# google/kubeflow

Measured on AMD Instinct MI355X. Metric: pytorchjob_train_tokens_per_s, higher is better.
Workload: dtype bf16; 1 GPU; model=llama3-8b, global_batch=7, seq_len=4096, parallelism=dp1

## Files before the change

kubeflow_amd/ops/__init__.py:

```python
from __future__ import annotations

import ctypes
import os
from typing import Optional

import torch

from . import reference
from . import _backend

__all__ = [
    "rms_norm", "layer_norm", "rope", "flash_attention", "attention_decode",
    "flash_attention_rect", "skinny_linear", "kv_store",
    "decode_rope_store", "skinny_linear_q8", "quantize_fp8_rows",
    "dequantize_fp8_rows",
    "cross_entropy", "fused_adamw", "rope_cos_sin", "native_available",
    "masked_attention",
    "swiglu", "fused_qkv_attention",
]

rope_cos_sin = reference.rope_cos_sin


def native_available() -> bool:
# ... 446 lines not shown
    def backward(ctx, dy):
        lib = _backend.require()
        (h2,) = ctx.saved_tensors
        T, F2 = h2.shape
        dy2 = dy.contiguous().view(T, F2 // 2)
        dh = torch.empty_like(h2)
        _backend.check(lib.kf_swiglu_bwd(_p(dh), _p(dy2), _p(h2), T, F2 // 2,
                                         _stream()), "swiglu_bwd")
        return dh.view(ctx.shape)


def swiglu(h: torch.Tensor) -> torch.Tensor:
    if _use_native(h):
        return _SwigluHip.apply(h)
    g, u = h.chunk(2, dim=-1)
    return torch.nn.functional.silu(g) * u



class _FusedQkvAttentionHip(torch.autograd.Function):

    @staticmethod
    def forward(ctx, qkv, cos, sin, Hq, Hkv, D, causal, scale):
        lib = _backend.require()
        B, S, _ = qkv.shape
        ts = (Hq + 2 * Hkv) * D
        qkv = qkv.contiguous()
        _backend.check(
            lib.kf_rope(_p(qkv), _p_off(qkv, Hq * D), _fp(cos), _fp(sin),
                        _ip_or_null(None), B, S, Hq, Hkv, D, ts, ts, 0, 0,
                        _stream()), "rope_fwd")
        o = torch.empty(B, S, Hq * D, dtype=qkv.dtype, device=qkv.device)
        lse = torch.empty(B, Hq, S, dtype=torch.float32, device=qkv.device)
        _backend.check(
            lib.kf_attn_fwd(_p(o), _fp(lse), _p(qkv), _p_off(qkv, Hq * D),
                            _p_off(qkv, (Hq + Hkv) * D), B, S, Hq, Hkv, D,
                            ts, ts, float(scale), int(causal), _stream()),
            "attn_fwd")
        ctx.save_for_backward(qkv, cos, sin, o, lse)
        ctx.meta = (Hq, Hkv, D, causal, scale)
        return o

    @staticmethod
    def backward(ctx, dout):
        lib = _backend.require()
        qkv, cos, sin, o, lse = ctx.saved_tensors
        Hq, Hkv, D, causal, scale = ctx.meta
        B, S, _ = qkv.shape
        ts = (Hq + 2 * Hkv) * D
        dout = dout.contiguous()
        dqkv = torch.empty_like(qkv)
        delta = torch.empty(B, Hq, S, dtype=torch.float32, device=qkv.device)
        _backend.check(
            lib.kf_attn_bwd(_p(dqkv), _p_off(dqkv, Hq * D),
                            _p_off(dqkv, (Hq + Hkv) * D), _p(dout), _p(qkv),
                            _p_off(qkv, Hq * D), _p_off(qkv, (Hq + Hkv) * D),
                            _p(o), _fp(lse), _fp(delta), B, S, Hq, Hkv, D,
                            ts, ts, ts, ts, float(scale), int(causal),
                            _stream()), "attn_bwd")
        _backend.check(
            lib.kf_rope(_p(dqkv), _p_off(dqkv, Hq * D), _fp(cos), _fp(sin),
                        _ip_or_null(None), B, S, Hq, Hkv, D, ts, ts, 0, 1,
                        _stream()), "rope_bwd")
        return dqkv, None, None, None, None, None, None, None


def fused_qkv_attention(qkv: torch.Tensor, cos: torch.Tensor,
                        sin: torch.Tensor, Hq: int, Hkv: int, D: int,
                        causal: bool = True,
                        scale: Optional[float] = None) -> torch.Tensor:
    if scale is None:
        scale = D ** -0.5
    B, S, _ = qkv.shape
    if _use_native(qkv) and S % 128 == 0:
        return _FusedQkvAttentionHip.apply(qkv, cos, sin, Hq, Hkv, D, causal,
                                           scale)
    q, k, v = qkv.split([Hq * D, Hkv * D, Hkv * D], dim=-1)
    q = q.reshape(B, S, Hq, D)
    k = k.reshape(B, S, Hkv, D)
    v = v.reshape(B, S, Hkv, D)
    q, k = rope(q, k, cos, sin)
    o = flash_attention(q, k, v, causal=causal, scale=scale)
    return o.reshape(B, S, Hq * D)



class _LayerNormHip(torch.autograd.Function):
    @staticmethod
    def forward(ctx, x, weight, bias, eps):
        lib = _backend.require()
        shape = x.shape
        x2 = x.contiguous().view(-1, shape[-1])
        rows, cols = x2.shape
        y = torch.empty_like(x2)
        mu = torch.empty(rows, dtype=torch.float32, device=x.device)
        rstd = torch.empty(rows, dtype=torch.float32, device=x.device)
        _backend.check(
            lib.kf_layernorm_fwd(_p(y), _fp(mu), _fp(rstd), _p(x2), _p(weight),
                                 _p(bias), rows, cols, float(eps), _stream()),
            "layernorm_fwd")
        ctx.save_for_backward(x2, weight, mu, rstd)
        ctx.shape = shape
        return y.view(shape)

    @staticmethod
    def backward(ctx, dy):
        lib = _backend.require()
        x2, weight, mu, rstd = ctx.saved_tensors
        rows, cols = x2.shape
        dy2 = dy.contiguous().view(rows, cols)
        dx = torch.empty_like(x2)
        dw = torch.empty_like(weight)
        db = torch.empty_like(weight)
        part = torch.zeros(2 * cols, dtype=torch.float32, device=x2.device)
        _backend.check(
            lib.kf_layernorm_bwd(_p(dx), _p(dw), _p(db), _fp(part), _p(dy2),
# ... 120 lines not shown
```

kubeflow_amd/ops/_backend.py:

```python
from __future__ import annotations

import ctypes
import os
from pathlib import Path

_LIB_PATH = Path(__file__).resolve().parent / "libkfops.so"
_lib = None
_load_error: str | None = None


def native_enabled() -> bool:
    return os.environ.get("KF_NATIVE_KERNELS", "1") != "0"


def try_load():
    global _lib, _load_error
    if _lib is not None:
        return _lib
    if not native_enabled():
        _load_error = "disabled via KF_NATIVE_KERNELS=0"
        return None
    from . import build_ext
    if build_ext.needs_build():
        try:
# ... 13 lines not shown
def require():
    lib = try_load()
    if lib is None:
        raise RuntimeError(
            "kubeflow_amd native kernels unavailable on a GPU machine: "
            f"{_load_error}. Build with `python -m kubeflow_amd.ops.build_ext` "
            "or set KF_NATIVE_KERNELS=0 to explicitly allow the (slow) "
            "reference path.")
    return lib


def _configure(lib: ctypes.CDLL) -> None:
    c = ctypes
    P, F, I64, I32, FP = c.c_void_p, c.c_float, c.c_int64, c.c_int, c.POINTER(c.c_float)
    PI64 = c.POINTER(c.c_int64)
    PI32 = c.POINTER(c.c_int32)
    lib.kf_rmsnorm_fwd.restype = I32
    lib.kf_rmsnorm_fwd.argtypes = [P, FP, P, P, I64, I64, F, P]
    lib.kf_rmsnorm_bwd.restype = I32
    lib.kf_rmsnorm_bwd.argtypes = [P, P, FP, P, P, P, FP, I64, I64, P]
    lib.kf_rmsnorm_bwd_nparts.restype = I64
    lib.kf_rmsnorm_bwd_nparts.argtypes = [I64]
    lib.kf_rope.restype = I32
    lib.kf_rope.argtypes = [P, P, FP, FP, PI64, I64, I64, I64, I64, I64, I64, I64, I64, I32, P]
    lib.kf_adamw.restype = I32
    lib.kf_adamw.argtypes = [P, FP, P, FP, FP, FP, I64, F, F, F, F, F, I64, P]
    lib.kf_ce_fwd.restype = I32
    lib.kf_ce_fwd.argtypes = [FP, FP, P, PI64, I64, I64, I64, P]
    lib.kf_ce_bwd.restype = I32
    lib.kf_ce_bwd.argtypes = [P, P, FP, PI64, FP, I64, I64, I64, P]
    lib.kf_attn_fwd.restype = I32
    lib.kf_attn_fwd.argtypes = [P, FP, P, P, P, I64, I64, I64, I64, I64, I64, I64, F, I32, P]
    if hasattr(lib, "kf_skinny_gemm"):
        lib.kf_skinny_gemm.restype = I32
        lib.kf_skinny_gemm.argtypes = [P, P, P, P, FP, F, I64, I64, I64,
                                       I64, I64, I64, I64, P]
    if hasattr(lib, "kf_skinny_gemm_q8"):
        lib.kf_skinny_gemm_q8.restype = I32
        lib.kf_skinny_gemm_q8.argtypes = [P, P, P, FP, P, FP, F, I64,
                                          I64, I64, I64, I64, I64, I64,
                                          P]
    if hasattr(lib, "kf_kv_store"):
        lib.kf_kv_store.restype = I32
        lib.kf_kv_store.argtypes = [P, P, P, P, P, P, I64, I64, I64, P]
    if hasattr(lib, "kf_attn_fwd4_rect"):
        lib.kf_attn_fwd4_rect.restype = I32
        lib.kf_attn_fwd4_rect.argtypes = [P, FP, P, P, P, I64, I64, I64,
                                          I64, I64, I64, I64, I64, F, I64, P]
    if hasattr(lib, "kf_attn_bwd"):
        lib.kf_attn_bwd.restype = I32
        lib.kf_attn_bwd.argtypes = [P, P, P, P, P, P, P, P, FP, FP, I64, I64,
                                    I64, I64, I64, I64, I64, I64, I64, F, I32,
                                    P]
    lib.kf_layernorm_fwd.restype = I32
    lib.kf_layernorm_fwd.argtypes = [P, FP, FP, P, P, P, I64, I64, F, P]
    lib.kf_layernorm_bwd.restype = I32
    lib.kf_layernorm_bwd.argtypes = [P, P, P, FP, P, P, P, FP, FP, I64, I64, P]
    lib.kf_layernorm_bwd_nparts.restype = I64
    lib.kf_layernorm_bwd_nparts.argtypes = [I64]
    lib.kf_swiglu_fwd.restype = I32
    lib.kf_swiglu_fwd.argtypes = [P, P, I64, I64, P]
    lib.kf_swiglu_bwd.restype = I32
    lib.kf_swiglu_bwd.argtypes = [P, P, P, I64, I64, P]
    lib.kf_attn_decode.restype = I32
    lib.kf_attn_decode.argtypes = [P, P, P, P, P, P, PI32, PI32, I64, I64,
                                   I64, I64, I64, I64, F, P]
    if hasattr(lib, "kf_decode_rope_store"):
        lib.kf_decode_rope_store.restype = I32
        lib.kf_decode_rope_store.argtypes = [P, P, P, P, FP, FP, PI32, P,
                                             I64, I64, I64, I64, I64, P]


def check(err: int, name: str) -> None:
    if err != 0:
        raise RuntimeError(f"HIP kernel {name} failed with hipError_t={err}")
```

kubeflow_amd/ops/csrc/attention_bwd.hip:

```cpp

#include "kf_common.h"

typedef __bf16 kf_bf16x8 __attribute__((ext_vector_type(8)));
typedef float kf_f32x4 __attribute__((ext_vector_type(4)));

#define AB_D 128

__device__ __forceinline__ int kf_swz2(int row, int byte_in_row, int row_bytes,
                                       int xor_mask) {
  return row * row_bytes + (byte_in_row ^ ((row & xor_mask) << 4));
}

__global__ __launch_bounds__(256) void kf_attn_delta2_kernel(
    float* __restrict__ delta, const unsigned short* __restrict__ dout,
    const unsigned short* __restrict__ o, int64_t B, int S, int Hq) {
  const int64_t nrows = B * (int64_t)S * Hq;
  const int wid = threadIdx.x / KF_WAVE;
  const int lane = threadIdx.x & (KF_WAVE - 1);
  for (int64_t row = blockIdx.x * 4 + wid; row < nrows; row += gridDim.x * 4) {
    const unsigned short* dor = dout + row * AB_D;
    const unsigned short* orow = o + row * AB_D;
    kf_short4 a = *reinterpret_cast<const kf_short4*>(dor + lane * 2);
    kf_short4 bv = *reinterpret_cast<const kf_short4*>(orow + lane * 2);
    float s = kf_bf16_to_f32((unsigned short)a[0]) *
// ... 251 lines not shown
                        : __expf(st[nt][r] * scale - lse_c);
          float ds = p * (dpt[nt][r] - dlt_c) * scale;
          const int prow = lg * 4 + r;
          *reinterpret_cast<unsigned short*>(
              pt_lds[w] + kf_swz2(prow, (nt * 16 + l16) * 2, 64, 3)) =
              kf_f32_to_bf16(p);
          *reinterpret_cast<unsigned short*>(
              dst_lds[w] + kf_swz2(prow, (nt * 16 + l16) * 2, 64, 3)) =
              kf_f32_to_bf16(ds);
        }
      }
      __builtin_amdgcn_s_waitcnt(0);

      kf_bf16x8 ptf = *reinterpret_cast<const kf_bf16x8*>(
          pt_lds[w] + kf_swz2(l16, lg * 16, 64, 3));
      kf_bf16x8 dstf = *reinterpret_cast<const kf_bf16x8*>(
          dst_lds[w] + kf_swz2(l16, lg * 16, 64, 3));
#pragma unroll
      for (int nt = 0; nt < 8; ++nt) {
        kf_bf16x8 dob = *reinterpret_cast<const kf_bf16x8*>(
            dot_lds + kf_swz2(nt * 16 + l16, lg * 16, 64, 3));
        dvacc[nt] =
            __builtin_amdgcn_mfma_f32_16x16x32_bf16(ptf, dob, dvacc[nt], 0, 0, 0);
        kf_bf16x8 qb = *reinterpret_cast<const kf_bf16x8*>(
            qt_lds + kf_swz2(nt * 16 + l16, lg * 16, 64, 3));
        dkacc[nt] =
            __builtin_amdgcn_mfma_f32_16x16x32_bf16(dstf, qb, dkacc[nt], 0, 0, 0);
      }
    }
  }

  const int krow0 = kt * 64 + w * 16 + lg * 4;
#pragma unroll
  for (int r = 0; r < 4; ++r) {
    const int64_t base = (b * S + krow0 + r) * dkts + (int64_t)hkv * AB_D;
#pragma unroll
    for (int nt = 0; nt < 8; ++nt) {
      dk[base + nt * 16 + l16] = kf_f32_to_bf16(dkacc[nt][r]);
      dv[base + nt * 16 + l16] = kf_f32_to_bf16(dvacc[nt][r]);
    }
  }
}

extern "C" int kf_attn_bwd8_dq(void*, const void*, const void*, const void*,
                               const void*, const float*, const float*,
                               int64_t, int64_t, int64_t, int64_t, int64_t,
                               int64_t, int64_t, float, int, void*);
extern "C" int kf_attn_bwd8_dkv(void*, void*, const void*, const void*,
                                const void*, const void*, const float*,
                                const float*, int64_t, int64_t, int64_t,
                                int64_t, int64_t, int64_t, int64_t, float,
                                int, void*);

KF_EXPORT int kf_attn_bwd(void* dq, void* dk, void* dv, const void* dout,
                          const void* q, const void* k, const void* v,
                          const void* o, const float* lse, float* delta,
                          int64_t B, int64_t S, int64_t Hq, int64_t Hkv,
                          int64_t D, int64_t qts, int64_t kts, int64_t dqts,
                          int64_t dkts, float scale, int causal,
                          void* stream) {
  if (D != AB_D || S % 64 || Hq % Hkv) return (int)hipErrorInvalidValue;
  if (qts == 0) qts = Hq * AB_D;
  if (kts == 0) kts = Hkv * AB_D;
  if (dqts == 0) dqts = Hq * AB_D;
  if (dkts == 0) dkts = Hkv * AB_D;
  hipLaunchKernelGGL(kf_attn_delta2_kernel,
                     dim3(kf_grid_for(B * S * Hq, 4)), dim3(256), 0,
                     (hipStream_t)stream, delta, (const unsigned short*)dout,
                     (const unsigned short*)o, B, (int)S, (int)Hq);
  int err = (int)hipGetLastError();
  if (err) return err;
  if (S % 256 == 0) {
    err = kf_attn_bwd8_dq(dq, q, k, v, dout, lse, delta, B, S, Hq, Hkv, qts,
                          kts, dqts, scale, causal, stream);
    if (err) return err;
    return kf_attn_bwd8_dkv(dk, dv, q, k, v, dout, lse, delta, B, S, Hq, Hkv,
                            qts, kts, dkts, scale, causal, stream);
  }
  dim3 gq((unsigned)(S / 64), (unsigned)Hq, (unsigned)B);
  hipLaunchKernelGGL(kf_attn_dq_kernel, gq, dim3(256), 0, (hipStream_t)stream,
                     (unsigned short*)dq, (const unsigned short*)q,
                     (const unsigned short*)k, (const unsigned short*)v,
                     (const unsigned short*)dout, lse, delta, B, (int)S,
                     (int)Hq, (int)Hkv, qts, kts, dqts, scale, causal);
  err = (int)hipGetLastError();
  if (err) return err;
  dim3 gkv((unsigned)(S / 64), (unsigned)Hkv, (unsigned)B);
  hipLaunchKernelGGL(kf_attn_dkv_kernel, gkv, dim3(256), 0,
                     (hipStream_t)stream, (unsigned short*)dk,
                     (unsigned short*)dv, (const unsigned short*)q,
                     (const unsigned short*)k, (const unsigned short*)v,
                     (const unsigned short*)dout, lse, delta, B, (int)S,
                     (int)Hq, (int)Hkv, qts, kts, dkts, scale, causal);
  return (int)hipGetLastError();
}
```

kubeflow_amd/ops/csrc/attention_bwd8.hip:

```cpp

#include "kf_common.h"

typedef __bf16 kf_bf16x8 __attribute__((ext_vector_type(8)));
typedef float kf_f32x16 __attribute__((ext_vector_type(16)));
typedef short kf_short4b __attribute__((ext_vector_type(4)));

#define AB_D 128
#define AB_LOG2E 1.44269504f

__device__ __forceinline__ int kf_vsub8(int r, int d) {
  return ((d >> 4) << 10) + ((r >> 2) << 6) + ((r & 3) << 4) + (d & 15);
}

__device__ __forceinline__ int kf_subrow8(int r, int byte_in_row) {
  return 2 * kf_vsub8(r, byte_in_row >> 1);
}

__device__ __forceinline__ unsigned int kf_cvt_pk_bf16b(float lo, float hi) {
  unsigned int r;
  asm volatile("v_cvt_pk_bf16_f32 %0, %1, %2" : "=v"(r) : "v"(lo), "v"(hi));
  return r;
}

__device__ __forceinline__ float kf_exp2b(float x) {
  float r;
  asm volatile("v_exp_f32 %0, %1" : "=v"(r) : "v"(x));
  return r;
}

#define KF_TR16_B(dst, addr, OFFLIT)                                    \
  asm volatile("ds_read_b64_tr_b16 %0, %1 offset:" OFFLIT               \
               : "=v"(dst) : "v"(addr))

__device__ __forceinline__ kf_bf16x8 kf_exchange8(const kf_f32x16& a,
                                                  int base) {
  unsigned int w0 = kf_cvt_pk_bf16b(a[base + 0], a[base + 1]);
  unsigned int w1 = kf_cvt_pk_bf16b(a[base + 2], a[base + 3]);
  unsigned int w2 = kf_cvt_pk_bf16b(a[base + 4], a[base + 5]);
  unsigned int w3 = kf_cvt_pk_bf16b(a[base + 6], a[base + 7]);
  auto s02 = __builtin_amdgcn_permlane32_swap(w0, w2, false, false);
  auto s13 = __builtin_amdgcn_permlane32_swap(w1, w3, false, false);
  unsigned int u[4] = {(unsigned)s02[0], (unsigned)s13[0], (unsigned)s02[1],
                       (unsigned)s13[1]};
  return *reinterpret_cast<kf_bf16x8*>(u);
}

__device__ __forceinline__ unsigned kf_tr_lane_off(int lane) {
  const int g = lane >> 4;
  return (unsigned)(((g & 1) << 11) + ((g >> 1) << 8) + ((lane & 15) << 3));
}

#define KF_TR_ACC_LOOP(acc, vbase, pb0, pb1)                                 \
  {                                                                          \
    kf_short4b t_[2][4];                                                     \
    KF_TR16_B(t_[0][0], (vbase), "0");                                       \
    KF_TR16_B(t_[0][1], (vbase), "128");                                     \
    KF_TR16_B(t_[0][2], (vbase), "512");                                     \
    KF_TR16_B(t_[0][3], (vbase), "640");                                     \
    _Pragma("unroll") for (int dt = 0; dt < 4; ++dt) {                       \
      if (dt < 3) {                                                          \
        const unsigned va_ = (vbase) + ((dt + 1) << 12);                     \
        KF_TR16_B(t_[(dt + 1) & 1][0], va_, "0");                            \
        KF_TR16_B(t_[(dt + 1) & 1][1], va_, "128");                          \
        KF_TR16_B(t_[(dt + 1) & 1][2], va_, "512");                          \
        KF_TR16_B(t_[(dt + 1) & 1][3], va_, "640");                          \
        asm volatile("s_waitcnt lgkmcnt(4)" ::: "memory");                   \
      } else {                                                               \
        asm volatile("s_waitcnt lgkmcnt(0)" ::: "memory");                   \
      }                                                                      \
      __builtin_amdgcn_sched_barrier(0);                                     \
      kf_short8 f0_ = __builtin_shufflevector(t_[dt & 1][0], t_[dt & 1][1],  \
                                              0, 1, 2, 3, 4, 5, 6, 7);       \
      kf_short8 f1_ = __builtin_shufflevector(t_[dt & 1][2], t_[dt & 1][3],  \
                                              0, 1, 2, 3, 4, 5, 6, 7);       \
      __builtin_amdgcn_s_setprio(1);                                         \
      acc[dt] = __builtin_amdgcn_mfma_f32_32x32x16_bf16(                     \
          *reinterpret_cast<kf_bf16x8*>(&f0_), (pb0), acc[dt], 0, 0, 0);     \
      acc[dt] = __builtin_amdgcn_mfma_f32_32x32x16_bf16(                     \
          *reinterpret_cast<kf_bf16x8*>(&f1_), (pb1), acc[dt], 0, 0, 0);     \
      __builtin_amdgcn_s_setprio(0);                                         \
    }                                                                        \
  }

#define KF_TR_ACC_LOOP_B(acc, vbase, pa0, pa1)                               \
  {                                                                          \
    kf_short4b t_[2][4];                                                     \
    KF_TR16_B(t_[0][0], (vbase), "0");                                       \
    KF_TR16_B(t_[0][1], (vbase), "128");                                     \
    KF_TR16_B(t_[0][2], (vbase), "512");                                     \
    KF_TR16_B(t_[0][3], (vbase), "640");                                     \
    _Pragma("unroll") for (int dt = 0; dt < 4; ++dt) {                       \
      if (dt < 3) {                                                          \
        const unsigned va_ = (vbase) + ((dt + 1) << 12);                     \
        KF_TR16_B(t_[(dt + 1) & 1][0], va_, "0");                            \
        KF_TR16_B(t_[(dt + 1) & 1][1], va_, "128");                          \
        KF_TR16_B(t_[(dt + 1) & 1][2], va_, "512");                          \
        KF_TR16_B(t_[(dt + 1) & 1][3], va_, "640");                          \
        asm volatile("s_waitcnt lgkmcnt(4)" ::: "memory");                   \
      } else {                                                               \
        asm volatile("s_waitcnt lgkmcnt(0)" ::: "memory");                   \
      }                                                                      \
      __builtin_amdgcn_sched_barrier(0);                                     \
      kf_short8 f0_ = __builtin_shufflevector(t_[dt & 1][0], t_[dt & 1][1],  \
                                              0, 1, 2, 3, 4, 5, 6, 7);       \
      kf_short8 f1_ = __builtin_shufflevector(t_[dt & 1][2], t_[dt & 1][3],  \
                                              0, 1, 2, 3, 4, 5, 6, 7);       \
      __builtin_amdgcn_s_setprio(1);                                         \
      acc[dt] = __builtin_amdgcn_mfma_f32_32x32x16_bf16(                     \
          (pa0), *reinterpret_cast<kf_bf16x8*>(&f0_), acc[dt], 0, 0, 0);     \
      acc[dt] = __builtin_amdgcn_mfma_f32_32x32x16_bf16(                     \
          (pa1), *reinterpret_cast<kf_bf16x8*>(&f1_), acc[dt], 0, 0, 0);     \
      __builtin_amdgcn_s_setprio(0);                                         \
    }                                                                        \
  }

#define DQ8_QT 256
#define DQ8_KT 64

__global__ __launch_bounds__(512, 2) void kf_attn_dq8_kernel(
    unsigned short* __restrict__ dq, const unsigned short* __restrict__ q,
    const unsigned short* __restrict__ k, const unsigned short* __restrict__ v,
    const unsigned short* __restrict__ dout, const float* __restrict__ lse,
    const float* __restrict__ delta, int64_t B, int S, int Hq, int Hkv,
    int64_t qts, int64_t kts, int64_t dqts, float scale, int causal) {
  __shared__ unsigned char k_lds[2][DQ8_KT * AB_D * 2];
  __shared__ unsigned char v_lds[2][DQ8_KT * AB_D * 2];

  const int nqt = gridDim.x / (Hq * (int)B);
  const int qt = causal ? (nqt - 1 - blockIdx.x / (Hq * (int)B))
                        : (int)(blockIdx.x / (Hq * (int)B));
  const int rest = blockIdx.x % (Hq * (int)B);
  const int hq = rest % Hq;
  const int64_t b = rest / Hq;
  const int hkv = hq / (Hq / Hkv);
  const int tid = threadIdx.x;
  const int w = tid / KF_WAVE;
  const int lane = tid & 63, l31 = lane & 31, hi = lane >> 5;
  const int qrow_g = qt * DQ8_QT + w * 32 + l31;
  const int wave_qmax = qt * DQ8_QT + w * 32 + 31;
  const float scale2 = scale * AB_LOG2E;

  kf_bf16x8 qfrag[8], dofrag[8];
  {
    const int64_t qb = (b * S + qrow_g) * qts + (int64_t)hq * AB_D;
    const int64_t db = ((b * S + qrow_g) * (int64_t)Hq + hq) * AB_D;
#pragma unroll
    for (int kk = 0; kk < 8; ++kk) {
      qfrag[kk] =
          *reinterpret_cast<const kf_bf16x8*>(q + qb + kk * 16 + hi * 8);
      dofrag[kk] =
          *reinterpret_cast<const kf_bf16x8*>(dout + db + kk * 16 + hi * 8);
    }
  }
  const float lse2_q =
      lse[(b * Hq + hq) * (int64_t)S + qrow_g] * AB_LOG2E;
  const float dlt_q = delta[(b * Hq + hq) * (int64_t)S + qrow_g];

  kf_f32x16 dqacc[4];
#pragma unroll
  for (int i = 0; i < 4; ++i) dqacc[i] = kf_f32x16{0.f};

  const unsigned short* kg0 = k + (b * S) * kts + (int64_t)hkv * AB_D;
  const unsigned short* vg0 = v + (b * S) * kts + (int64_t)hkv * AB_D;
  const int sr0 = tid >> 4, sr1 = (tid + 512) >> 4, c8 = tid & 15;
  const unsigned tr_off = kf_tr_lane_off(lane);

  const int last_kt =
      causal ? (qt * DQ8_QT + DQ8_QT - 1) / DQ8_KT : (S / DQ8_KT - 1);

  kf_short8 kst0, kst1, vst0, vst1;
  kst0 = *reinterpret_cast<const kf_short8*>(kg0 + sr0 * kts + c8 * 8);
  kst1 = *reinterpret_cast<const kf_short8*>(kg0 + sr1 * kts + c8 * 8);
  vst0 = *reinterpret_cast<const kf_short8*>(vg0 + sr0 * kts + c8 * 8);
  vst1 = *reinterpret_cast<const kf_short8*>(vg0 + sr1 * kts + c8 * 8);
  *reinterpret_cast<kf_short8*>(k_lds[0] + 2 * kf_vsub8(sr0, c8 * 8)) = kst0;
  *reinterpret_cast<kf_short8*>(k_lds[0] + 2 * kf_vsub8(sr1, c8 * 8)) = kst1;
  *reinterpret_cast<kf_short8*>(v_lds[0] + 2 * kf_vsub8(sr0, c8 * 8)) = vst0;
// ... 17 lines not shown
      const int kv_lo = kt * DQ8_KT + mt * 32;
      if (causal && kv_lo > wave_qmax) continue;
      kf_f32x16 st = kf_f32x16{0.f}, dpt = kf_f32x16{0.f};
      __builtin_amdgcn_s_setprio(1);
#pragma unroll
      for (int kk = 0; kk < 8; ++kk) {
        kf_bf16x8 ka = *reinterpret_cast<const kf_bf16x8*>(
            k_lds[cur] + kf_subrow8(mt * 32 + l31, kk * 32 + hi * 16));
        st = __builtin_amdgcn_mfma_f32_32x32x16_bf16(ka, qfrag[kk], st, 0, 0,
                                                     0);
        kf_bf16x8 va = *reinterpret_cast<const kf_bf16x8*>(
            v_lds[cur] + kf_subrow8(mt * 32 + l31, kk * 32 + hi * 16));
        dpt = __builtin_amdgcn_mfma_f32_32x32x16_bf16(va, dofrag[kk], dpt, 0,
                                                      0, 0);
      }
      __builtin_amdgcn_s_setprio(0);

      const int kv0 = kv_lo + hi * 4;
      const bool need_mask = causal && kv_lo + 31 > qt * DQ8_QT + w * 32;
      if (need_mask) {
#pragma unroll
        for (int r = 0; r < 16; ++r) {
          const int kv = kv0 + (r & 3) + 8 * (r >> 2);
          const float p = (kv > qrow_g)
                              ? 0.f
                              : kf_exp2b(st[r] * scale2 - lse2_q);
          st[r] = p * (dpt[r] - dlt_q) * scale;
        }
      } else {
#pragma unroll
        for (int r = 0; r < 16; ++r) {
          const float p = kf_exp2b(st[r] * scale2 - lse2_q);
          st[r] = p * (dpt[r] - dlt_q) * scale;
        }
      }
      kf_bf16x8 pb0 = kf_exchange8(st, 0), pb1 = kf_exchange8(st, 8);
      const unsigned vbase =
          (unsigned)(size_t)(k_lds[cur]) + tr_off + (mt << 10);
      KF_TR_ACC_LOOP(dqacc, vbase, pb0, pb1);
    }

    if (have_next) {
      const int nxt = cur ^ 1;
      *reinterpret_cast<kf_short8*>(k_lds[nxt] + 2 * kf_vsub8(sr0, c8 * 8)) =
          kst0;
      *reinterpret_cast<kf_short8*>(k_lds[nxt] + 2 * kf_vsub8(sr1, c8 * 8)) =
          kst1;
      *reinterpret_cast<kf_short8*>(v_lds[nxt] + 2 * kf_vsub8(sr0, c8 * 8)) =
          vst0;
      *reinterpret_cast<kf_short8*>(v_lds[nxt] + 2 * kf_vsub8(sr1, c8 * 8)) =
          vst1;
    }
    __syncthreads();
  }

  const int64_t dqb = (b * S + qrow_g) * dqts + (int64_t)hq * AB_D;
#pragma unroll
  for (int dt = 0; dt < 4; ++dt)
#pragma unroll
    for (int rq = 0; rq < 4; ++rq) {
      const int d0 = dt * 32 + 8 * rq + 4 * hi;
      unsigned short q4[4];
#pragma unroll
      for (int j = 0; j < 4; ++j)
        q4[j] = kf_f32_to_bf16(dqacc[dt][rq * 4 + j]);
      *reinterpret_cast<kf_short4b*>(dq + dqb + d0) =
          *reinterpret_cast<kf_short4b*>(q4);
    }
}

#define DKV8_KT 256
#define DKV8_QT 64

__global__ __launch_bounds__(512, 2) void kf_attn_dv8_kernel(
    unsigned short* __restrict__ dv, const unsigned short* __restrict__ q,
    const unsigned short* __restrict__ k,
    const unsigned short* __restrict__ dout, const float* __restrict__ lse,
    int64_t B, int S, int Hq, int Hkv, int64_t qts, int64_t kts,
    int64_t dkts, float scale, int causal) {
  __shared__ unsigned char q_lds[2][DKV8_QT * AB_D * 2];
  __shared__ unsigned char dot_lds[2][DKV8_QT * AB_D * 2];
  __shared__ float lse_s[2][DKV8_QT];

  const int kt = blockIdx.x / (Hkv * (int)B);
  const int rest = blockIdx.x % (Hkv * (int)B);
  const int hkv = rest % Hkv;
  const int64_t b = rest / Hkv;
  const int g = Hq / Hkv;
  const int tid = threadIdx.x;
  const int w = tid / KF_WAVE;
  const int lane = tid & 63, l31 = lane & 31, hi = lane >> 5;
  const int kvrow_g = kt * DKV8_KT + w * 32 + l31;
  const int wave_kv_min = kt * DKV8_KT + w * 32;
  const float scale2 = scale * AB_LOG2E;

  const unsigned short* kvb_k =
      k + (b * S + kvrow_g) * kts + (int64_t)hkv * AB_D;
  kf_bf16x8 kbf[8];
#pragma unroll
  for (int kk = 0; kk < 8; ++kk)
    kbf[kk] =
        *reinterpret_cast<const kf_bf16x8*>(kvb_k + kk * 16 + hi * 8);

  kf_f32x16 dvacc[4];
#pragma unroll
  for (int i = 0; i < 4; ++i) dvacc[i] = kf_f32x16{0.f};
// ... 52 lines not shown
      __builtin_amdgcn_s_setprio(1);
#pragma unroll
      for (int kk = 0; kk < 8; ++kk) {
        kf_bf16x8 qa = *reinterpret_cast<const kf_bf16x8*>(
            q_lds[cur] + kf_subrow8(mt * 32 + l31, kk * 32 + hi * 16));
        sacc = __builtin_amdgcn_mfma_f32_32x32x16_bf16(qa, kbf[kk], sacc, 0,
                                                       0, 0);
      }
      __builtin_amdgcn_s_setprio(0);

      const int q0 = mt * 32 + hi * 4;
      const bool need_mask = causal && q_lo <= kt * DKV8_KT + w * 32 + 31;
      if (need_mask) {
#pragma unroll
        for (int r = 0; r < 16; ++r) {
          const int ql = q0 + (r & 3) + 8 * (r >> 2);
          const int qq = qt * DKV8_QT + ql;
          sacc[r] = (kvrow_g > qq)
                        ? 0.f
                        : kf_exp2b(sacc[r] * scale2 - lse_s[cur][ql]);
        }
      } else {
#pragma unroll
        for (int r = 0; r < 16; ++r) {
          const int ql = q0 + (r & 3) + 8 * (r >> 2);
          sacc[r] = kf_exp2b(sacc[r] * scale2 - lse_s[cur][ql]);
        }
      }
      kf_bf16x8 pa0 = kf_exchange8(sacc, 0), pa1 = kf_exchange8(sacc, 8);
      const unsigned vbase =
          (unsigned)(size_t)(dot_lds[cur]) + tr_off + (mt << 10);
      KF_TR_ACC_LOOP_B(dvacc, vbase, pa0, pa1);
    }
    if (have_next) stage_write(cur ^ 1);
    __syncthreads();
  }

  const int kvbase = kt * DKV8_KT + w * 32 + hi * 4;
#pragma unroll
  for (int r = 0; r < 16; ++r) {
    const int kvr = kvbase + (r & 3) + 8 * (r >> 2);
    const int64_t base = (b * S + kvr) * dkts + (int64_t)hkv * AB_D;
#pragma unroll
    for (int dt = 0; dt < 4; ++dt)
      dv[base + dt * 32 + l31] = kf_f32_to_bf16(dvacc[dt][r]);
  }
}

__global__ __launch_bounds__(512, 2) void kf_attn_dk8_kernel(
    unsigned short* __restrict__ dk, const unsigned short* __restrict__ q,
    const unsigned short* __restrict__ k, const unsigned short* __restrict__ v,
    const unsigned short* __restrict__ dout, const float* __restrict__ lse,
    const float* __restrict__ delta, int64_t B, int S, int Hq, int Hkv,
    int64_t qts, int64_t kts, int64_t dkts, float scale, int causal) {
  __shared__ unsigned char q_lds[2][DKV8_QT * AB_D * 2];
  __shared__ unsigned char do_lds[2][DKV8_QT * AB_D * 2];
  __shared__ float lse_s2[2][DKV8_QT], dlt_s2[2][DKV8_QT];

  const int kt = blockIdx.x / (Hkv * (int)B);
  const int rest = blockIdx.x % (Hkv * (int)B);
  const int hkv = rest % Hkv;
  const int64_t b = rest / Hkv;
  const int g = Hq / Hkv;
  const int tid = threadIdx.x;
  const int w = tid / KF_WAVE;
  const int lane = tid & 63, l31 = lane & 31, hi = lane >> 5;
  const int kvrow_g = kt * DKV8_KT + w * 32 + l31;
  const int wave_kv_min = kt * DKV8_KT + w * 32;
  const float scale2 = scale * AB_LOG2E;

  const unsigned short* kvb_k =
      k + (b * S + kvrow_g) * kts + (int64_t)hkv * AB_D;
  const unsigned short* kvb_v =
      v + (b * S + kvrow_g) * kts + (int64_t)hkv * AB_D;
  kf_bf16x8 kbf[8], vbf[8];
#pragma unroll
  for (int kk = 0; kk < 8; ++kk) {
    kbf[kk] =
        *reinterpret_cast<const kf_bf16x8*>(kvb_k + kk * 16 + hi * 8);
    vbf[kk] =
        *reinterpret_cast<const kf_bf16x8*>(kvb_v + kk * 16 + hi * 8);
  }

  kf_f32x16 dkacc[4];
#pragma unroll
  for (int i = 0; i < 4; ++i) dkacc[i] = kf_f32x16{0.f};

  const int qt0 = causal ? (kt * DKV8_KT) / DKV8_QT : 0;
  const int nqt = S / DKV8_QT;
  const int per_head = nqt - qt0;
  const int total = g * per_head;
  const int sr0 = tid >> 4, sr1 = (tid + 512) >> 4, c8 = tid & 15;
  const unsigned tr_off = kf_tr_lane_off(lane);

  kf_short8 sq0, sq1, sd0, sd1;
  float lse_ld = 0.f, dlt_ld = 0.f;
  auto stage_load = [&](int flat) {
    const int hq = hkv * g + flat / per_head;
    const int qt = qt0 + flat % per_head;
    const unsigned short* qg =
        q + (b * S + qt * DKV8_QT) * qts + (int64_t)hq * AB_D;
    const unsigned short* dog =
        dout + ((b * S + qt * DKV8_QT) * (int64_t)Hq + hq) * AB_D;
    if (tid < DKV8_QT)
      lse_ld = lse[(b * Hq + hq) * (int64_t)S + qt * DKV8_QT + tid];
    else if (tid < 2 * DKV8_QT)
      dlt_ld =
// ... 31 lines not shown
    for (int mt = 0; mt < 2; ++mt) {
      const int q_lo = qt * DKV8_QT + mt * 32;
      if (causal && q_lo + 31 < wave_kv_min) continue;
      kf_f32x16 sacc = kf_f32x16{0.f}, dpacc = kf_f32x16{0.f};
      __builtin_amdgcn_s_setprio(1);
#pragma unroll
      for (int kk = 0; kk < 8; ++kk) {
        kf_bf16x8 qa = *reinterpret_cast<const kf_bf16x8*>(
            q_lds[cur] + kf_subrow8(mt * 32 + l31, kk * 32 + hi * 16));
        sacc = __builtin_amdgcn_mfma_f32_32x32x16_bf16(qa, kbf[kk], sacc, 0,
                                                       0, 0);
        kf_bf16x8 da = *reinterpret_cast<const kf_bf16x8*>(
            do_lds[cur] + kf_subrow8(mt * 32 + l31, kk * 32 + hi * 16));
        dpacc = __builtin_amdgcn_mfma_f32_32x32x16_bf16(da, vbf[kk], dpacc,
                                                        0, 0, 0);
      }
      __builtin_amdgcn_s_setprio(0);

      const int q0 = mt * 32 + hi * 4;
      const bool need_mask = causal && q_lo <= kt * DKV8_KT + w * 32 + 31;
      if (need_mask) {
#pragma unroll
        for (int r = 0; r < 16; ++r) {
          const int ql = q0 + (r & 3) + 8 * (r >> 2);
          const int qq = qt * DKV8_QT + ql;
          const float p =
              (kvrow_g > qq)
                  ? 0.f
                  : kf_exp2b(sacc[r] * scale2 - lse_s2[cur][ql]);
          sacc[r] = p * (dpacc[r] - dlt_s2[cur][ql]) * scale;
        }
      } else {
#pragma unroll
        for (int r = 0; r < 16; ++r) {
          const int ql = q0 + (r & 3) + 8 * (r >> 2);
          const float p = kf_exp2b(sacc[r] * scale2 - lse_s2[cur][ql]);
          sacc[r] = p * (dpacc[r] - dlt_s2[cur][ql]) * scale;
        }
      }
      kf_bf16x8 ds0 = kf_exchange8(sacc, 0), ds1 = kf_exchange8(sacc, 8);
      const unsigned vbase =
          (unsigned)(size_t)(q_lds[cur]) + tr_off + (mt << 10);
      KF_TR_ACC_LOOP_B(dkacc, vbase, ds0, ds1);
    }
    if (have_next) stage_write(cur ^ 1);
    __syncthreads();
  }

  const int kvbase = kt * DKV8_KT + w * 32 + hi * 4;
#pragma unroll
  for (int r = 0; r < 16; ++r) {
    const int kvr = kvbase + (r & 3) + 8 * (r >> 2);
    const int64_t base = (b * S + kvr) * dkts + (int64_t)hkv * AB_D;
#pragma unroll
    for (int dt = 0; dt < 4; ++dt)
      dk[base + dt * 32 + l31] = kf_f32_to_bf16(dkacc[dt][r]);
  }
}

KF_EXPORT int kf_attn_bwd8_dq(void* dq, const void* q, const void* k,
                              const void* v, const void* dout,
                              const float* lse, const float* delta, int64_t B,
                              int64_t S, int64_t Hq, int64_t Hkv, int64_t qts,
                              int64_t kts, int64_t dqts, float scale,
                              int causal, void* stream) {
  dim3 gq((unsigned)((S / DQ8_QT) * Hq * B), 1, 1);
  hipLaunchKernelGGL(kf_attn_dq8_kernel, gq, dim3(512), 0,
                     (hipStream_t)stream, (unsigned short*)dq,
                     (const unsigned short*)q, (const unsigned short*)k,
                     (const unsigned short*)v, (const unsigned short*)dout,
                     lse, delta, B, (int)S, (int)Hq, (int)Hkv, qts, kts, dqts,
                     scale, causal);
  return (int)hipGetLastError();
}

KF_EXPORT int kf_attn_bwd8_dkv(void* dk, void* dv, const void* q,
                               const void* k, const void* v, const void* dout,
                               const float* lse, const float* delta,
                               int64_t B, int64_t S, int64_t Hq, int64_t Hkv,
                               int64_t qts, int64_t kts, int64_t dkts,
                               float scale, int causal, void* stream) {
  dim3 gkv((unsigned)((S / DKV8_KT) * Hkv * B), 1, 1);
  hipLaunchKernelGGL(kf_attn_dv8_kernel, gkv, dim3(512), 0,
                     (hipStream_t)stream, (unsigned short*)dv,
                     (const unsigned short*)q, (const unsigned short*)k,
                     (const unsigned short*)dout, lse, B, (int)S, (int)Hq,
                     (int)Hkv, qts, kts, dkts, scale, causal);
  int err = (int)hipGetLastError();
  if (err) return err;
  hipLaunchKernelGGL(kf_attn_dk8_kernel, gkv, dim3(512), 0,
                     (hipStream_t)stream, (unsigned short*)dk,
                     (const unsigned short*)q, (const unsigned short*)k,
                     (const unsigned short*)v, (const unsigned short*)dout,
                     lse, delta, B, (int)S, (int)Hq, (int)Hkv, qts, kts,
                     dkts, scale, causal);
  return (int)hipGetLastError();
}
```

Baseline: 21070 tokens/s.

## Fuse RoPE backward into attention backward and merge dK/dV kernels

Applies the inverse RoPE rotation to dQ and dK inside the attention backward epilogues, which removes the separate rope backward kernel and its extra read/write pass over dqkv. It also adds a fused dK+dV kernel, now the default, that computes S and dP once per tile and accumulates both gradients. Previously two separate kernels each recomputed the QK^T products and reloaded Q/dO. The fused kernel keeps V in LDS and uses more registers (launch bounds of 2), so occupancy may drop. An environment variable switches back to the old split path.

```diff
diff --git a/kubeflow_amd/ops/__init__.py b/kubeflow_amd/ops/__init__.py
--- a/kubeflow_amd/ops/__init__.py
+++ b/kubeflow_amd/ops/__init__.py
@@ -522,16 +522,14 @@
         dqkv = torch.empty_like(qkv)
         delta = torch.empty(B, Hq, S, dtype=torch.float32, device=qkv.device)
         _backend.check(
-            lib.kf_attn_bwd(_p(dqkv), _p_off(dqkv, Hq * D),
-                            _p_off(dqkv, (Hq + Hkv) * D), _p(dout), _p(qkv),
-                            _p_off(qkv, Hq * D), _p_off(qkv, (Hq + Hkv) * D),
-                            _p(o), _fp(lse), _fp(delta), B, S, Hq, Hkv, D,
-                            ts, ts, ts, ts, float(scale), int(causal),
-                            _stream()), "attn_bwd")
-        _backend.check(
-            lib.kf_rope(_p(dqkv), _p_off(dqkv, Hq * D), _fp(cos), _fp(sin),
-                        _ip_or_null(None), B, S, Hq, Hkv, D, ts, ts, 0, 1,
-                        _stream()), "rope_bwd")
+            lib.kf_attn_bwd_rope(_p(dqkv), _p_off(dqkv, Hq * D),
+                                 _p_off(dqkv, (Hq + Hkv) * D), _p(dout),
+                                 _p(qkv), _p_off(qkv, Hq * D),
+                                 _p_off(qkv, (Hq + Hkv) * D), _p(o),
+                                 _fp(lse), _fp(delta), B, S, Hq, Hkv, D,
+                                 ts, ts, ts, ts, float(scale), int(causal),
+                                 _fp(cos), _fp(sin), 0, _stream()),
+            "attn_bwd_rope")
         return dqkv, None, None, None, None, None, None, None
 
 
diff --git a/kubeflow_amd/ops/_backend.py b/kubeflow_amd/ops/_backend.py
--- a/kubeflow_amd/ops/_backend.py
+++ b/kubeflow_amd/ops/_backend.py
@@ -89,6 +89,21 @@
         lib.kf_attn_bwd.argtypes = [P, P, P, P, P, P, P, P, FP, FP, I64, I64,
                                     I64, I64, I64, I64, I64, I64, I64, F, I32,
                                     P]
+    if hasattr(lib, "kf_attn_bwd_rope"):
+        lib.kf_attn_bwd_rope.restype = I32
+        lib.kf_attn_bwd_rope.argtypes = [P, P, P, P, P, P, P, P, FP, FP, I64,
+                                         I64, I64, I64, I64, I64, I64, I64,
+                                         I64, F, I32, FP, FP, I64, P]
+    dq8 = [P, P, P, P, P, FP, FP, I64, I64, I64, I64, I64, I64, I64, F, I32]
+    dkv8 = [P] + dq8
+    for name, args in (("kf_attn_bwd8_dq", dq8), ("kf_attn_bwd8_dkv", dkv8),
+                       ("kf_attn_bwd8_dkv_fused", dkv8)):
+        if hasattr(lib, name):
+            getattr(lib, name).restype = I32
+            getattr(lib, name).argtypes = args + [P]
+        if hasattr(lib, name + "_rope"):
+            getattr(lib, name + "_rope").restype = I32
+            getattr(lib, name + "_rope").argtypes = args + [FP, FP, I64, P]
     lib.kf_layernorm_fwd.restype = I32
     lib.kf_layernorm_fwd.argtypes = [P, FP, FP, P, P, P, I64, I64, F, P]
     lib.kf_layernorm_bwd.restype = I32
diff --git a/kubeflow_amd/ops/csrc/attention_bwd.hip b/kubeflow_amd/ops/csrc/attention_bwd.hip
--- a/kubeflow_amd/ops/csrc/attention_bwd.hip
+++ b/kubeflow_amd/ops/csrc/attention_bwd.hip
@@ -327,6 +327,49 @@
                                 int64_t, int64_t, int64_t, int64_t, float,
                                 int, void*);
 
+extern "C" int kf_attn_bwd8_dq_rope(void*, const void*, const void*,
+                                    const void*, const void*, const float*,
+                                    const float*, int64_t, int64_t, int64_t,
+                                    int64_t, int64_t, int64_t, int64_t, float,
+                                    int, const float*, const float*, int64_t,
+                                    void*);
+extern "C" int kf_attn_bwd8_dkv_rope(void*, void*, const void*, const void*,
+                                     const void*, const void*, const float*,
+                                     const float*, int64_t, int64_t, int64_t,
+                                     int64_t, int64_t, int64_t, int64_t,
+                                     float, int, const float*, const float*,
+                                     int64_t, void*);
+extern "C" int kf_attn_bwd8_dkv_fused_rope(void*, void*, const void*,
+                                           const void*, const void*,
+                                           const void*, const float*,
+                                           const float*, int64_t, int64_t,
+                                           int64_t, int64_t, int64_t, int64_t,
+                                           int64_t, float, int, const float*,
+                                           const float*, int64_t, void*);
+
+extern "C" int kf_rope(void*, void*, const float*, const float*,
+                       const int64_t*, int64_t, int64_t, int64_t, int64_t,
+                       int64_t, int64_t, int64_t, int64_t, int, void*);
+
+static int kf_attn_bwd_impl() {
+  static int cached = -1;
+  if (cached < 0) {
+    const char* e = getenv("KF_ATTN_BWD_IMPL");
+    cached = (e && e[0] == '1') ? 1 : 2;
+  }
+  return cached;
+}
+
+KF_EXPORT int kf_attn_bwd_rope(void* dq, void* dk, void* dv, const void* dout,
+                               const void* q, const void* k, const void* v,
+                               const void* o, const float* lse, float* delta,
+                               int64_t B, int64_t S, int64_t Hq, int64_t Hkv,
+                               int64_t D, int64_t qts, int64_t kts,
+                               int64_t dqts, int64_t dkts, float scale,
+                               int causal, const float* cost,
+                               const float* sint, int64_t pos_offset,
+                               void* stream);
+
 KF_EXPORT int kf_attn_bwd(void* dq, void* dk, void* dv, const void* dout,
                           const void* q, const void* k, const void* v,
                           const void* o, const float* lse, float* delta,
@@ -334,7 +377,22 @@
                           int64_t D, int64_t qts, int64_t kts, int64_t dqts,
                           int64_t dkts, float scale, int causal,
                           void* stream) {
+  return kf_attn_bwd_rope(dq, dk, dv, dout, q, k, v, o, lse, delta, B, S, Hq,
+                          Hkv, D, qts, kts, dqts, dkts, scale, causal,
+                          nullptr, nullptr, 0, stream);
+}
+
+KF_EXPORT int kf_attn_bwd_rope(void* dq, void* dk, void* dv, const void* dout,
+                               const void* q, const void* k, const void* v,
+                               const void* o, const float* lse, float* delta,
+                               int64_t B, int64_t S, int64_t Hq, int64_t Hkv,
+                               int64_t D, int64_t qts, int64_t kts,
+                               int64_t dqts, int64_t dkts, float scale,
+                               int causal, const float* cost,
+                               const float* sint, int64_t pos_offset,
+                               void* stream) {
   if (D != AB_D || S % 64 || Hq % Hkv) return (int)hipErrorInvalidValue;
+  if ((cost == nullptr) != (sint == nullptr)) return (int)hipErrorInvalidValue;
   if (qts == 0) qts = Hq * AB_D;
   if (kts == 0) kts = Hkv * AB_D;
   if (dqts == 0) dqts = Hq * AB_D;
@@ -346,11 +404,18 @@
   int err = (int)hipGetLastError();
   if (err) return err;
   if (S % 256 == 0) {
-    err = kf_attn_bwd8_dq(dq, q, k, v, dout, lse, delta, B, S, Hq, Hkv, qts,
-                          kts, dqts, scale, causal, stream);
+    err = kf_attn_bwd8_dq_rope(dq, q, k, v, dout, lse, delta, B, S, Hq, Hkv,
+                               qts, kts, dqts, scale, causal, cost, sint,
+                               pos_offset, stream);
     if (err) return err;
-    return kf_attn_bwd8_dkv(dk, dv, q, k, v, dout, lse, delta, B, S, Hq, Hkv,
-                            qts, kts, dkts, scale, causal, stream);
+    if (kf_attn_bwd_impl() == 1)
+      return kf_attn_bwd8_dkv_rope(dk, dv, q, k, v, dout, lse, delta, B, S,
+                                   Hq, Hkv, qts, kts, dkts, scale, causal,
+                                   cost, sint, pos_offset, stream);
+    return kf_attn_bwd8_dkv_fused_rope(dk, dv, q, k, v, dout, lse, delta, B,
+                                       S, Hq, Hkv, qts, kts, dkts, scale,
+                                       causal, cost, sint, pos_offset,
+                                       stream);
   }
   dim3 gq((unsigned)(S / 64), (unsigned)Hq, (unsigned)B);
   hipLaunchKernelGGL(kf_attn_dq_kernel, gq, dim3(256), 0, (hipStream_t)stream,
@@ -367,5 +432,8 @@
                      (const unsigned short*)k, (const unsigned short*)v,
                      (const unsigned short*)dout, lse, delta, B, (int)S,
                      (int)Hq, (int)Hkv, qts, kts, dkts, scale, causal);
-  return (int)hipGetLastError();
-}
+  err = (int)hipGetLastError();
+  if (err || !cost) return err;
+  return kf_rope(dq, dk, cost, sint, nullptr, B, S, Hq, Hkv, D, dqts, dkts,
+                 pos_offset, 1, stream);
+}
diff --git a/kubeflow_amd/ops/csrc/attention_bwd8.hip b/kubeflow_amd/ops/csrc/attention_bwd8.hip
--- a/kubeflow_amd/ops/csrc/attention_bwd8.hip
+++ b/kubeflow_amd/ops/csrc/attention_bwd8.hip
@@ -49,6 +49,15 @@
   const int g = lane >> 4;
   return (unsigned)(((g & 1) << 11) + ((g >> 1) << 8) + ((lane & 15) << 3));
 }
+
+#define KF_ROPE_ADJ_PAIR(x1, x2, c, s)                                \
+  {                                                                   \
+    const float a_ = kf_bf16_to_f32(kf_f32_to_bf16(x1));              \
+    const float b_ = kf_bf16_to_f32(kf_f32_to_bf16(x2));              \
+    const float t1_ = b_ * (s), t2_ = a_ * (s);                       \
+    (x1) = __builtin_fmaf(a_, (c), t1_);                              \
+    (x2) = __builtin_fmaf(b_, (c), -t2_);                             \
+  }
 
 #define KF_TR_ACC_LOOP(acc, vbase, pb0, pb1)                                 \
   {                                                                          \
@@ -122,7 +131,9 @@
     const unsigned short* __restrict__ k, const unsigned short* __restrict__ v,
     const unsigned short* __restrict__ dout, const float* __restrict__ lse,
     const float* __restrict__ delta, int64_t B, int S, int Hq, int Hkv,
-    int64_t qts, int64_t kts, int64_t dqts, float scale, int causal) {
+    int64_t qts, int64_t kts, int64_t dqts, float scale, int causal,
+    const float* __restrict__ cost, const float* __restrict__ sint,
+    int64_t pos_offset) {
   __shared__ unsigned char k_lds[2][DQ8_KT * AB_D * 2];
   __shared__ unsigned char v_lds[2][DQ8_KT * AB_D * 2];
 
@@ -246,6 +257,23 @@
           vst1;
     }
     __syncthreads();
+  }
+
+  if (cost) {
+    const int64_t cb = (pos_offset + qrow_g) * (AB_D / 2) + 4 * hi;
+#pragma unroll
+    for (int dt = 0; dt < 2; ++dt)
+#pragma unroll
+      for (int rq = 0; rq < 4; ++rq) {
+        const kf_float4 c4 =
+            *reinterpret_cast<const kf_float4*>(cost + cb + dt * 32 + 8 * rq);
+        const kf_float4 s4 =
+            *reinterpret_cast<const kf_float4*>(sint + cb + dt * 32 + 8 * rq);
+#pragma unroll
+        for (int j = 0; j < 4; ++j)
+          KF_ROPE_ADJ_PAIR(dqacc[dt][rq * 4 + j], dqacc[dt + 2][rq * 4 + j],
+                           c4[j], s4[j]);
+      }
   }
 
   const int64_t dqb = (b * S + qrow_g) * dqts + (int64_t)hq * AB_D;
@@ -404,7 +432,9 @@
     const unsigned short* __restrict__ k, const unsigned short* __restrict__ v,
     const unsigned short* __restrict__ dout, const float* __restrict__ lse,
     const float* __restrict__ delta, int64_t B, int S, int Hq, int Hkv,
-    int64_t qts, int64_t kts, int64_t dkts, float scale, int causal) {
+    int64_t qts, int64_t kts, int64_t dkts, float scale, int causal,
+    const float* __restrict__ cost, const float* __restrict__ sint,
+    int64_t pos_offset) {
   __shared__ unsigned char q_lds[2][DKV8_QT * AB_D * 2];
   __shared__ unsigned char do_lds[2][DKV8_QT * AB_D * 2];
   __shared__ float lse_s2[2][DKV8_QT], dlt_s2[2][DKV8_QT];
@@ -542,10 +572,222 @@
   for (int r = 0; r < 16; ++r) {
     const int kvr = kvbase + (r & 3) + 8 * (r >> 2);
     const int64_t base = (b * S + kvr) * dkts + (int64_t)hkv * AB_D;
+    if (cost) {
+      const int64_t cb = (pos_offset + kvr) * (AB_D / 2) + l31;
+#pragma unroll
+      for (int dt = 0; dt < 2; ++dt)
+        KF_ROPE_ADJ_PAIR(dkacc[dt][r], dkacc[dt + 2][r], cost[cb + dt * 32],
+                         sint[cb + dt * 32]);
+    }
 #pragma unroll
     for (int dt = 0; dt < 4; ++dt)
       dk[base + dt * 32 + l31] = kf_f32_to_bf16(dkacc[dt][r]);
   }
+}
+
+#define DKVF_WAVES 8
+#define DKVF_THREADS (DKVF_WAVES * KF_WAVE)
+#define DKVF_KT (DKVF_WAVES * 32)
+#define DKVF_NST (DKV8_QT * 16 / DKVF_THREADS)
+#define DKVF_SLAB (DKV8_QT * 16 * 2)
+
+__global__ __launch_bounds__(DKVF_THREADS, 2) void kf_attn_dkv8f_kernel(
+    unsigned short* __restrict__ dk, unsigned short* __restrict__ dv,
+    const unsigned short* __restrict__ q, const unsigned short* __restrict__ k,
+    const unsigned short* __restrict__ v,
+    const unsigned short* __restrict__ dout, const float* __restrict__ lse,
+    const float* __restrict__ delta, int64_t B, int S, int Hq, int Hkv,
+    int64_t qts, int64_t kts, int64_t dkts, float scale, int causal,
+    const float* __restrict__ cost, const float* __restrict__ sint,
+    int64_t pos_offset) {
+  __shared__ unsigned char q_lds[2][DKV8_QT * AB_D * 2];
+  __shared__ unsigned char do_lds[2][DKV8_QT * AB_D * 2];
+  __shared__ float lse_s3[2][DKV8_QT], dlt_s3[2][DKV8_QT];
+  __shared__ unsigned char v_lds[DKVF_WAVES / 2][DKV8_QT * AB_D * 2];
+
+  const int kt = blockIdx.x / (Hkv * (int)B);
+  const int rest = blockIdx.x % (Hkv * (int)B);
+  const int hkv = rest % Hkv;
+  const int64_t b = rest / Hkv;
+  const int g = Hq / Hkv;
+  const int tid = threadIdx.x;
+  const int w = tid / KF_WAVE;
+  const int lane = tid & 63, l31 = lane & 31, hi = lane >> 5;
+  const int kvrow_g = kt * DKVF_KT + w * 32 + l31;
+  const int wave_kv_min = kt * DKVF_KT + w * 32;
+  const float scale2 = scale * AB_LOG2E;
+
+  const unsigned short* kvb_k =
+      k + (b * S + kvrow_g) * kts + (int64_t)hkv * AB_D;
+  const unsigned short* kvb_v =
+      v + (b * S + kvrow_g) * kts + (int64_t)hkv * AB_D;
+  kf_bf16x8 kbf[8];
+  unsigned char* vfrag =
+      v_lds[w >> 1] + kf_subrow8((w & 1) * 32 + l31, hi * 16);
+#pragma unroll
+  for (int kk = 0; kk < 8; ++kk) {
+    kbf[kk] =
+        *reinterpret_cast<const kf_bf16x8*>(kvb_k + kk * 16 + hi * 8);
+    *reinterpret_cast<kf_bf16x8*>(vfrag + kk * DKVF_SLAB) =
+        *reinterpret_cast<const kf_bf16x8*>(kvb_v + kk * 16 + hi * 8);
+  }
+
+  kf_f32x16 dkacc[4], dvacc[4];
+#pragma unroll
+  for (int i = 0; i < 4; ++i) {
+    dkacc[i] = kf_f32x16{0.f};
+    dvacc[i] = kf_f32x16{0.f};
+  }
+
+  const int qt0 = causal ? (kt * DKVF_KT) / DKV8_QT : 0;
+  const int nqt = S / DKV8_QT;
+  const int per_head = nqt - qt0;
+  const int total = g * per_head;
+  const int c8 = tid & 15;
+  const unsigned tr_off = kf_tr_lane_off(lane);
+  constexpr int kRowsPerPass = DKVF_THREADS / 16;
+  const unsigned qoff = (unsigned)((tid >> 4) * (int)qts + c8 * 8);
+  const unsigned dooff = (unsigned)((tid >> 4) * Hq * AB_D + c8 * 8);
+
+  kf_short8 sq[DKVF_NST], sd[DKVF_NST];
+  float rc_ld = 0.f;
+  auto stage_load = [&](int flat) {
+    const int hq = hkv * g + flat / per_head;
+    const int qt = qt0 + flat % per_head;
+    const unsigned short* qg =
+        q + (b * S + qt * DKV8_QT) * qts + (int64_t)hq * AB_D;
+    const unsigned short* dog =
+        dout + ((b * S + qt * DKV8_QT) * (int64_t)Hq + hq) * AB_D;
+    if (tid < 2 * DKV8_QT) {
+      const float* rc = tid < DKV8_QT ? lse : delta;
+      rc_ld = rc[(b * Hq + hq) * (int64_t)S + qt * DKV8_QT +
+                 (tid & (DKV8_QT - 1))];
+    }
+#pragma unroll
+    for (int j = 0; j < DKVF_NST; ++j) {
+      sq[j] = *reinterpret_cast<const kf_short8*>(
+          qg + j * kRowsPerPass * qts + qoff);
+      sd[j] = *reinterpret_cast<const kf_short8*>(
+          dog + j * kRowsPerPass * (int64_t)Hq * AB_D + dooff);
+    }
+  };
+  auto stage_write = [&](int buf) {
+    if (tid < DKV8_QT) lse_s3[buf][tid] = rc_ld * AB_LOG2E;
+    else if (tid < 2 * DKV8_QT) dlt_s3[buf][tid - DKV8_QT] = rc_ld;
+#pragma unroll
+    for (int j = 0; j < DKVF_NST; ++j) {
+      const int sr = (tid + j * DKVF_THREADS) >> 4;
+      *reinterpret_cast<kf_short8*>(q_lds[buf] + 2 * kf_vsub8(sr, c8 * 8)) =
+          sq[j];
+      *reinterpret_cast<kf_short8*>(do_lds[buf] + 2 * kf_vsub8(sr, c8 * 8)) =
+          sd[j];
+    }
+  };
+
+  stage_load(0);
+  stage_write(0);
+  __syncthreads();
+  for (int flat = 0; flat < total; ++flat) {
+    const int cur = flat & 1;
+    const bool have_next = flat + 1 < total;
+    if (have_next) stage_load(flat + 1);
+    const int qt = qt0 + flat % per_head;
+
+#pragma unroll
+    for (int mt = 0; mt < 2; ++mt) {
+      const int q_lo = qt * DKV8_QT + mt * 32;
+      if (causal && q_lo + 31 < wave_kv_min) continue;
+      kf_f32x16 sacc = kf_f32x16{0.f}, dpacc = kf_f32x16{0.f};
+      __builtin_amdgcn_s_setprio(1);
+#pragma unroll
+      for (int kk = 0; kk < 8; ++kk) {
+        kf_bf16x8 qa = *reinterpret_cast<const kf_bf16x8*>(
+            q_lds[cur] + kf_subrow8(mt * 32 + l31, kk * 32 + hi * 16));
+        sacc = __builtin_amdgcn_mfma_f32_32x32x16_bf16(qa, kbf[kk], sacc, 0,
+                                                       0, 0);
+        kf_bf16x8 da = *reinterpret_cast<const kf_bf16x8*>(
+            do_lds[cur] + kf_subrow8(mt * 32 + l31, kk * 32 + hi * 16));
+        kf_bf16x8 vb =
+            *reinterpret_cast<const kf_bf16x8*>(vfrag + kk * DKVF_SLAB);
+        dpacc = __builtin_amdgcn_mfma_f32_32x32x16_bf16(da, vb, dpacc, 0, 0,
+                                                        0);
+      }
+      __builtin_amdgcn_s_setprio(0);
+
+      const int q0 = mt * 32 + hi * 4;
+      const bool need_mask = causal && q_lo <= kt * DKVF_KT + w * 32 + 31;
+      if (need_mask) {
+#pragma unroll
+        for (int r = 0; r < 16; ++r) {
+          const int ql = q0 + (r & 3) + 8 * (r >> 2);
+          const int qq = qt * DKV8_QT + ql;
+          sacc[r] = (kvrow_g > qq)
+                        ? 0.f
+                        : kf_exp2b(sacc[r] * scale2 - lse_s3[cur][ql]);
+        }
+      } else {
+#pragma unroll
+        for (int r = 0; r < 16; ++r) {
+          const int ql = q0 + (r & 3) + 8 * (r >> 2);
+          sacc[r] = kf_exp2b(sacc[r] * scale2 - lse_s3[cur][ql]);
+        }
+      }
+      kf_bf16x8 pa0 = kf_exchange8(sacc, 0), pa1 = kf_exchange8(sacc, 8);
+#pragma unroll
+      for (int r = 0; r < 16; ++r) {
+        const int ql = q0 + (r & 3) + 8 * (r >> 2);
+        sacc[r] = sacc[r] * (dpacc[r] - dlt_s3[cur][ql]) * scale;
+      }
+      kf_bf16x8 ds0 = kf_exchange8(sacc, 0), ds1 = kf_exchange8(sacc, 8);
+
+      const unsigned vbase_do =
+          (unsigned)(size_t)(do_lds[cur]) + tr_off + (mt << 10);
+      KF_TR_ACC_LOOP_B(dvacc, vbase_do, pa0, pa1);
+      const unsigned vbase_q =
+          (unsigned)(size_t)(q_lds[cur]) + tr_off + (mt << 10);
+      KF_TR_ACC_LOOP_B(dkacc, vbase_q, ds0, ds1);
+    }
+    if (have_next) stage_write(cur ^ 1);
+    __syncthreads();
+  }
+
+  const int kvbase = kt * DKVF_KT + w * 32 + hi * 4;
+#pragma unroll
+  for (int r = 0; r < 16; ++r) {
+    const int kvr = kvbase + (r & 3) + 8 * (r >> 2);
+    const int64_t base = (b * S + kvr) * dkts + (int64_t)hkv * AB_D;
+#pragma unroll
+    for (int dt = 0; dt < 4; ++dt)
+      dv[base + dt * 32 + l31] = kf_f32_to_bf16(dvacc[dt][r]);
+    if (cost) {
+      const int64_t cb = (pos_offset + kvr) * (AB_D / 2) + l31;
+#pragma unroll
+      for (int dt = 0; dt < 2; ++dt)
+        KF_ROPE_ADJ_PAIR(dkacc[dt][r], dkacc[dt + 2][r], cost[cb + dt * 32],
+                         sint[cb + dt * 32]);
+    }
+#pragma unroll
+    for (int dt = 0; dt < 4; ++dt)
+      dk[base + dt * 32 + l31] = kf_f32_to_bf16(dkacc[dt][r]);
+  }
+}
+
+KF_EXPORT int kf_attn_bwd8_dq_rope(void* dq, const void* q, const void* k,
+                                   const void* v, const void* dout,
+                                   const float* lse, const float* delta,
+                                   int64_t B, int64_t S, int64_t Hq,
+                                   int64_t Hkv, int64_t qts, int64_t kts,
+                                   int64_t dqts, float scale, int causal,
+                                   const float* cost, const float* sint,
+                                   int64_t pos_offset, void* stream) {
+  dim3 gq((unsigned)((S / DQ8_QT) * Hq * B), 1, 1);
+  hipLaunchKernelGGL(kf_attn_dq8_kernel, gq, dim3(512), 0,
+                     (hipStream_t)stream, (unsigned short*)dq,
+                     (const unsigned short*)q, (const unsigned short*)k,
+                     (const unsigned short*)v, (const unsigned short*)dout,
+                     lse, delta, B, (int)S, (int)Hq, (int)Hkv, qts, kts, dqts,
+                     scale, causal, cost, sint, pos_offset);
+  return (int)hipGetLastError();
 }
 
 KF_EXPORT int kf_attn_bwd8_dq(void* dq, const void* q, const void* k,
@@ -554,22 +796,20 @@
                               int64_t S, int64_t Hq, int64_t Hkv, int64_t qts,
                               int64_t kts, int64_t dqts, float scale,
                               int causal, void* stream) {
-  dim3 gq((unsigned)((S / DQ8_QT) * Hq * B), 1, 1);
-  hipLaunchKernelGGL(kf_attn_dq8_kernel, gq, dim3(512), 0,
-                     (hipStream_t)stream, (unsigned short*)dq,
-                     (const unsigned short*)q, (const unsigned short*)k,
-                     (const unsigned short*)v, (const unsigned short*)dout,
-                     lse, delta, B, (int)S, (int)Hq, (int)Hkv, qts, kts, dqts,
-                     scale, causal);
-  return (int)hipGetLastError();
-}
-
-KF_EXPORT int kf_attn_bwd8_dkv(void* dk, void* dv, const void* q,
-                               const void* k, const void* v, const void* dout,
-                               const float* lse, const float* delta,
-                               int64_t B, int64_t S, int64_t Hq, int64_t Hkv,
-                               int64_t qts, int64_t kts, int64_t dkts,
-                               float scale, int causal, void* stream) {
+  return kf_attn_bwd8_dq_rope(dq, q, k, v, dout, lse, delta, B, S, Hq, Hkv,
+                              qts, kts, dqts, scale, causal, nullptr, nullptr,
+                              0, stream);
+}
+
+KF_EXPORT int kf_attn_bwd8_dkv_rope(void* dk, void* dv, const void* q,
+                                    const void* k, const void* v,
+                                    const void* dout, const float* lse,
+                                    const float* delta, int64_t B, int64_t S,
+                                    int64_t Hq, int64_t Hkv, int64_t qts,
+                                    int64_t kts, int64_t dkts, float scale,
+                                    int causal, const float* cost,
+                                    const float* sint, int64_t pos_offset,
+                                    void* stream) {
   dim3 gkv((unsigned)((S / DKV8_KT) * Hkv * B), 1, 1);
   hipLaunchKernelGGL(kf_attn_dv8_kernel, gkv, dim3(512), 0,
                      (hipStream_t)stream, (unsigned short*)dv,
@@ -583,6 +823,47 @@
                      (const unsigned short*)q, (const unsigned short*)k,
                      (const unsigned short*)v, (const unsigned short*)dout,
                      lse, delta, B, (int)S, (int)Hq, (int)Hkv, qts, kts,
-                     dkts, scale, causal);
+                     dkts, scale, causal, cost, sint, pos_offset);
   return (int)hipGetLastError();
 }
+
+KF_EXPORT int kf_attn_bwd8_dkv(void* dk, void* dv, const void* q,
+                               const void* k, const void* v, const void* dout,
+                               const float* lse, const float* delta,
+                               int64_t B, int64_t S, int64_t Hq, int64_t Hkv,
+                               int64_t qts, int64_t kts, int64_t dkts,
+                               float scale, int causal, void* stream) {
+  return kf_attn_bwd8_dkv_rope(dk, dv, q, k, v, dout, lse, delta, B, S, Hq,
+                               Hkv, qts, kts, dkts, scale, causal, nullptr,
+                               nullptr, 0, stream);
+}
+
+KF_EXPORT int kf_attn_bwd8_dkv_fused_rope(
+    void* dk, void* dv, const void* q, const void* k, const void* v,
+    const void* dout, const float* lse, const float* delta, int64_t B,
+    int64_t S, int64_t Hq, int64_t Hkv, int64_t qts, int64_t kts,
+    int64_t dkts, float scale, int causal, const float* cost,
+    const float* sint, int64_t pos_offset, void* stream) {
+  if (S % DKVF_KT || Hq % Hkv) return (int)hipErrorInvalidValue;
+  dim3 gkv((unsigned)((S / DKVF_KT) * Hkv * B), 1, 1);
+  hipLaunchKernelGGL(kf_attn_dkv8f_kernel, gkv, dim3(DKVF_THREADS), 0,
+                     (hipStream_t)stream, (unsigned short*)dk,
+                     (unsigned short*)dv, (const unsigned short*)q,
+                     (const unsigned short*)k, (const unsigned short*)v,
+                     (const unsigned short*)dout, lse, delta, B, (int)S,
+                     (int)Hq, (int)Hkv, qts, kts, dkts, scale, causal, cost,
+                     sint, pos_offset);
+  return (int)hipGetLastError();
+}
+
+KF_EXPORT int kf_attn_bwd8_dkv_fused(void* dk, void* dv, const void* q,
+                                     const void* k, const void* v,
+                                     const void* dout, const float* lse,
+                                     const float* delta, int64_t B, int64_t S,
+                                     int64_t Hq, int64_t Hkv, int64_t qts,
+                                     int64_t kts, int64_t dkts, float scale,
+                                     int causal, void* stream) {
+  return kf_attn_bwd8_dkv_fused_rope(dk, dv, q, k, v, dout, lse, delta, B, S,
+                                     Hq, Hkv, qts, kts, dkts, scale, causal,
+                                     nullptr, nullptr, 0, stream);
+}
```

Result: faster. 21660 tokens/s, median of 6 (+2.8%).
